# zhouxuguang/GNXRayTracer

Hardware: AMD Instinct MI355X
Metric: Mrays/sec + wall-clock to 1024spp, dragon Cornell 1920×1080 (higher is better)
Workload: dtype f32; 1 GPU; cfg3: Cornell + synthetic 100000-tri mesh (stand-in for absent dragon.3d), Glass+Metal, PathIntegrator maxDepth 8 rr 1 spatial, Halton(1024), 1920x1080; passes_in_flight=4, sub_passes=56, spp_rendered=1024, gather=n/a, world_size=1, backend=none, devices_visible=1

## Files before the change

### gnxraytracer_amd/csrc/api.hip

```cpp
#include <hip/hip_runtime.h>

#include <chrono>
#include <cstdio>
#include <cstdlib>
#include <memory>
#include <mutex>
#include <string>
#include <thread>
#include <vector>

#include "host_scene.h"
#include "kernels.hip.h"
#include "trace4_kernel.hip.h"
#include "hlbvh_build.hip.h"
#include "refit_kernel.hip.h"
#include "material_kernel.hip.h"
#include "rebuild_kernel.hip.h"
#include "li_kernel.hip.h"
#include "views_kernel.hip.h"
#include "shade_query_kernel.hip.h"
#include "aov_kernel.hip.h"
#include "kernel_instances.h"

using namespace gnxr;
// ... 25 lines not shown
int gnxr_init(int device_id) {
    int n = 0;
    hipError_t e = hipGetDeviceCount(&n);
    if (e != hipSuccess || n <= 0) { set_error("no HIP device available; libgnxr has no CPU fallback"); return GNXR_ERR_NO_DEVICE; }
    if (device_id < 0 || device_id >= n) { set_error("device %d out of range (%d visible)", device_id, n); return GNXR_ERR_INVALID; }
    HIP_TRY(hipSetDevice(device_id));
    g_device = -1;
    g_devices.assign(1, device_id);
    g_peer_ok.assign(1, 1);
    return ensure_device();
}
int gnxr_init_devices(int32_t n_devices, const int32_t *device_ids) {
    if (n_devices <= 0 || n_devices > 64 || !device_ids) { set_error("bad device list"); return GNXR_ERR_INVALID; }
    int n = 0;
    hipError_t e = hipGetDeviceCount(&n);
    if (e != hipSuccess || n <= 0) { set_error("no HIP device available; libgnxr has no CPU fallback"); return GNXR_ERR_NO_DEVICE; }
    for (int i = 0; i < n_devices; ++i)
        if (device_ids[i] < 0 || device_ids[i] >= n) { set_error("device %d out of range (%d visible)", device_ids[i], n); return GNXR_ERR_INVALID; }
    int rc = gnxr_init(device_ids[0]);
    if (rc) return rc;
    g_devices.assign(device_ids, device_ids + n_devices);
    g_peer_ok.assign(n_devices, 1);
    for (int i = 1; i < n_devices; ++i) {
        if (device_ids[i] == device_ids[0]) continue;
        int can01 = 0, can10 = 0;
        bool ok = hipDeviceCanAccessPeer(&can01, device_ids[0], device_ids[i]) == hipSuccess && can01 &&
                  hipDeviceCanAccessPeer(&can10, device_ids[i], device_ids[0]) == hipSuccess && can10;
        if (ok) {
            hipError_t e0 = hipSetDevice(device_ids[0]) == hipSuccess ? hipDeviceEnablePeerAccess(device_ids[i], 0) : hipErrorInvalidDevice;
            hipError_t e1 = hipSetDevice(device_ids[i]) == hipSuccess ? hipDeviceEnablePeerAccess(device_ids[0], 0) : hipErrorInvalidDevice;
            ok = (e0 == hipSuccess || e0 == hipErrorPeerAccessAlreadyEnabled) && (e1 == hipSuccess || e1 == hipErrorPeerAccessAlreadyEnabled);
        }
        g_peer_ok[i] = ok ? 1 : 0;
        if (getenv("GNXR_VERBOSE")) fprintf(stderr, "[gnxr] device %d <-> %d: %s\n", device_ids[0], device_ids[i], ok ? "peer access" : "no peer access: rows are staged through the host");
    }
    (void)hipGetLastError();
    if (getenv("GNXR_NO_PEER")) for (int i = 1; i < n_devices; ++i) g_peer_ok[i] = 0;
    HIP_TRY(hipSetDevice(device_ids[0]));
    return GNXR_OK;
}
void gnxr_shutdown(void) { g_device = -1; g_devices.clear(); g_peer_ok.clear(); }
int gnxr_set_profiling(int flags) { g_profiling = flags; return GNXR_OK; }
#ifdef GX_SHADE_STATS
int gnxr_debug_shade_stats(unsigned long long *out16, int reset) {
    if (hipMemcpyFromSymbol(out16, HIP_SYMBOL(g_shade_stats), 16 * sizeof(unsigned long long)) != hipSuccess) return GNXR_ERR_INVALID;
    if (reset) { unsigned long long z[16] = {0}; (void)hipMemcpyToSymbol(HIP_SYMBOL(g_shade_stats), z, sizeof(z)); }
    return GNXR_OK;
}
#endif
#ifdef GX_TRACE_STATS
int gnxr_debug_trace_stats(unsigned long long *out16, int reset) {
    if (hipMemcpyFromSymbol(out16, HIP_SYMBOL(g_trace_stats), 24 * sizeof(unsigned long long)) != hipSuccess) return GNXR_ERR_INVALID;
    if (reset) { unsigned long long z[24] = {0}; (void)hipMemcpyToSymbol(HIP_SYMBOL(g_trace_stats), z, sizeof(z)); }
    return GNXR_OK;
}
#endif

static int upload_scene(gnxr_scene *s, size_t) {
    const CompiledScene &cs = s->cs;
    int rc;
    if (cs.bvh_max_depth + 1 > 64) { set_error("BVH depth %d exceeds the 64-entry traversal stack (BVHAccel.cpp:661)", cs.bvh_max_depth); return GNXR_ERR_UNSUPPORTED; }
    s->set_traversal(std::any_of(cs.nodes.begin(), cs.nodes.end(), [](const DNode &n) { return (n.meta & 0xffffu) > 127; }));
#define UP(field) if ((rc = s->field.upload(cs.field)) != GNXR_OK) return rc;
    UP(nodes) UP(nodes4) UP(tris) UP(leaf_boxes) UP(tri_class) UP(lights) UP(perms) UP(primes) UP(prime_sums) UP(prime_magic)
    UP(dmedia) UP(grid_density) UP(tri_media) UP(spheres) UP(textures) UP(tex_texels) UP(ewa_lut) UP(tri_uv) UP(tri_n) UP(tri_s)
    UP(aov_albedo)
    UP(env_texels4) UP(env_cond_func) UP(env_cond_cdf) UP(env_cond_int) UP(env_marg_func) UP(env_marg_cdf) UP(env_marg_guide) UP(env_cond_guide)
#undef UP
    {
        const size_t worst = 2 * cs.desc_materials.size();
        if ((rc = s->material_authored.alloc(worst)) || (rc = s->materials.alloc(1 + worst)) || (rc = s->materials_single.alloc(1 + worst))) return rc;
        if ((rc = s->material_authored.upload(cs.material_authored)) != GNXR_OK) return rc;
        const DTexTables rec = s->tex_tables(s->tri_uv.p, s->tri_n.p, s->tri_s.p);
        for (int k = 0; k < 2; ++k) {
            const std::vector<DMaterial> &src = k == 0 ? cs.materials : cs.materials_single;
            std::vector<DMaterial> up(src.size() + 1);
            memset(&up[0], 0, sizeof(DMaterial));
            memcpy(&up[0], &rec, sizeof(rec));
            std::copy(src.begin(), src.end(), up.begin() + 1);
            if ((rc = (k == 0 ? s->materials : s->materials_single).upload(up)) != GNXR_OK) return rc;
        }
    }
    if ((rc = s->infinite.upload(cs.infinite_lights)) != GNXR_OK) return rc;
    if ((rc = s->counters.alloc(1)) != GNXR_OK) return rc;
    if (hipHostMalloc((void **)&s->h_counters, sizeof(Counters)) != hipSuccess) { set_error("hipHostMalloc failed"); return GNXR_ERR_OOM; }
    if (hipHostMalloc((void **)&s->h_ring, sizeof(Counters) * gnxr_scene::kRing) != hipSuccess) { set_error("hipHostMalloc failed"); return GNXR_ERR_OOM; }
    for (hipEvent_t &e : s->ring_ev) HIP_TRY(hipEventCreateWithFlags(&e, hipEventDisableTiming));
    for (hipStream_t &a : s->aux_stream) HIP_TRY(hipStreamCreateWithFlags(&a, hipStreamNonBlocking));
    HIP_TRY(hipEventCreateWithFlags(&s->ev_fork, hipEventDisableTiming));
    for (hipEvent_t &e : s->ev_join) HIP_TRY(hipEventCreateWithFlags(&e, hipEventDisableTiming));
    return GNXR_OK;
}

int gnxr_scene_create(const gnxr_scene_desc *desc, gnxr_scene **out) {
    if (!desc || !out) { set_error("null argument"); return GNXR_ERR_INVALID; }
    int rc = ensure_device();
    if (rc) return rc;
    gnxr_scene *s = new (std::nothrow) gnxr_scene(g_device);
    if (!s) return GNXR_ERR_OOM;
    if (!compile_scene(desc, &s->cs, device_hlbvh_build)) { delete s; return GNXR_ERR_INVALID; }
    for (size_t i = 1; i < g_devices.size(); ++i) s->replicas.push_back(std::make_unique<gnxr_scene>(g_devices[i], s->host));
    if ((rc = s->each_copy(upload_scene)) != GNXR_OK) { delete s; return rc; }
    const CompiledScene &cs = s->cs;
    if (getenv("GNXR_VERBOSE"))
        fprintf(stderr, "[gnxr] scene: %zu tris, %zu nodes (depth %d), %zu 4-wide nodes (stack %d), wide=%d, %zu device(s)\n", cs.tris.size(), cs.nodes.size(), cs.bvh_max_depth,
                cs.nodes4.size(), cs.stack4_need, (int)s->wide_ok, s->n_copies());
// ... 282 lines not shown
```

### gnxraytracer_amd/csrc/api_render.hip.h

```cpp
#pragma once

struct TraceLaunch {
    int entries;
    int lds_entries;
    bool spill_needed;
    size_t lds;
    int n_top;
    int blocks;
};
static TraceLaunch trace_launch(const gnxr_scene *s, bool wide, bool spheres, long long total) {
    TraceLaunch t;
    t.entries = wide ? s->cs.stack4_need + 1 : s->cs.bvh_max_depth + 2;
    const int per_cu = g_trace_blocks_per_cu;
    const size_t fixed_b = wide ? (size_t)(kRayRecDwords + (spheres ? 1 : 0)) * kRqStride * sizeof(int) + (size_t)kTopCache * 128 + 128 : 0;
    t.lds_entries = std::min(std::min(t.entries, Knobs::trace_lds_levels()), std::max(2, (int)(((160 * 1024) / per_cu - 1024 - fixed_b) / (kBlock * sizeof(int)))));
    t.spill_needed = t.entries > t.lds_entries;
    t.lds = (size_t)t.lds_entries * kBlock * sizeof(int) + fixed_b;
    t.n_top = (int)std::min<size_t>(kTopCache, s->cs.root4 >= 0 ? s->cs.nodes4.size() : 0);
    t.blocks = (int)std::min<long long>((long long)g_num_cus * per_cu, (total + kBlock - 1) / kBlock);
    return t;
}

static int count_local_rows(const gnxr_render_params *p) {
    int rows = 0;
// ... 220 lines not shown
VolPackSet RenderState::pack_set(bool alt) {
    VolPackSet ps;
    if (!alt) {
        float4 *a[kVolPackF4] = {L.p, reinterpret_cast<float4 *>(vol_vs.p), vol_n1.p, vol_f.p, vol_Li.p, vol_Tr.p, vol_Ld.p, mis_Y.p, vol_mres.p};
        for (int i = 0; i < kVolPackF4; ++i) ps.f4[i] = a[i];
        record_ptrs(rec, ps.rec);
        ps.state = vol_state.p; ps.orig = vol_orig.p;
    } else {
        for (int i = 0; i < kVolPackF4; ++i) ps.f4[i] = vol_alt[i].p;
        record_ptrs(vol_alt_rec, ps.rec);
        ps.state = vol_alt_state.p; ps.orig = vol_alt_orig.p;
    }
    return ps;
}

struct RenderRun {
    gnxr_scene *s;
    RenderState &st;
    hipStream_t stream;
    const RenderPlan &pl;
    const RaySource *src;
    const ViewSource *views;
    DScene sc;
    DRender r;
    PathArrays pa;
    VolArrays va;
    WhittedArrays wa;
    DMediaTables mt;
    Counters *dctr;
    KernelTimer timer;
    const bool timing = (g_profiling & 1) != 0, count_wide = (g_profiling & 4) != 0, counting = (g_profiling & 2) != 0 && !count_wide;
    bool spheres;
    bool list_media = false;
    int n_lights, n_scene_media;
    unsigned long long rays_closest = 0, rays_any = 0, rays_mis = 0, media_segments = 0;
    unsigned long long new_paths = 0;
    unsigned int launches = 0, passes = 0, loop_iterations = 0;

    RenderRun(gnxr_scene *scene, hipStream_t stream_, const RenderPlan &plan, const RaySource *src_, const ViewSource *views_, const DScene &sc_, const DRender &r_)
        : s(scene), st(scene->st), stream(stream_), pl(plan), src(src_), views(views_), sc(sc_), r(r_), pa(st.path_arrays()), va(st.vol_arrays()),
          wa(st.whitted_arrays(plan, (int)scene->cs.desc_lights.size())), mt(scene->media_tables()), dctr(scene->counters.p), spheres(scene->cs.n_spheres > 0),
          n_lights((int)scene->cs.desc_lights.size()), n_scene_media((int)scene->cs.media.size()) {}

    void launch_trace(TraceWork w, int n_sh, int n_mis, bool count_rays = true);
    void compact(int mode, const int *qin, int nin, const unsigned char *keys, int nout, int nscatter, unsigned int *totals, int *o0, int *o1, int *o2, int *o3 = nullptr, int split = 0,
                 const unsigned *n_dev = nullptr);
    int shade_stage(const int *q_in, int n, int *q_out, const unsigned *n_dev);
    void raygen(const PathArrays &at, long long u0, int kk, unsigned char *medium_keys);
    void resolve(const PathArrays &at, long long u0, int kk);
    void bind_set(const VolPackSet &ps);
};

void RenderRun::launch_trace(TraceWork w, int n_sh, int n_mis, bool count_rays) {
    long long total = (long long)w.n_closest + 2ll * w.n_nee;
    if (total <= 0) return;
    w.order = nullptr;
    (void)hipMemsetAsync(&dctr->cursor, 0, sizeof(unsigned int), stream);
    const bool wide = s->wide_ok && !counting;
    const TraceLaunch tl = trace_launch(s, wide, spheres, total);
    if (timing) timer.begin(0, stream);
    const int chunk = Knobs::trace_chunk();
#define GX_TRACE(C, W, S) hipLaunchKernelGGL((k_trace<C, W, S>), dim3(tl.blocks), dim3(kBlock), tl.lds, stream, sc, pa, w, &dctr->cursor, dctr, tl.lds_entries, st.trace_spill.p, chunk)
#define GX_TRACE4(C, S, P) hipLaunchKernelGGL((k_trace4<C, S, P>), dim3(tl.blocks), dim3(kBlock), tl.lds, stream, sc, pa, w, &dctr->cursor, dctr, tl.lds_entries, st.trace_spill.p, chunk, tl.n_top)
#define GX_TRACE4_CS(C, S) do { if (tl.spill_needed) GX_TRACE4(C, S, true); else GX_TRACE4(C, S, false); } while (0)
    if (wide) {
        if (spheres) { if (count_wide) GX_TRACE4_CS(true, true); else GX_TRACE4_CS(false, true); }
        else { if (count_wide) GX_TRACE4_CS(true, false); else GX_TRACE4_CS(false, false); }
    } else {
        const bool cnt = counting || count_wide;
        if (spheres) { if (cnt) GX_TRACE(true, false, true); else GX_TRACE(false, false, true); }
        else { if (cnt) GX_TRACE(true, false, false); else GX_TRACE(false, false, false); }
    }
#undef GX_TRACE4_CS
#undef GX_TRACE4
#undef GX_TRACE
    if (timing) timer.end(stream);
    if (count_rays) {
        rays_closest += (unsigned long long)w.n_closest + (unsigned long long)n_mis;
        rays_any += (unsigned long long)n_sh;
        rays_mis += (unsigned long long)n_mis;
    }
    ++launches;
}

void RenderRun::compact(int mode, const int *qin, int nin, const unsigned char *keys, int nout, int nscatter, unsigned int *totals, int *o0, int *o1, int *o2, int *o3, int split,
                        const unsigned *n_dev) {
    const int tiles = (nin + kCompactTile - 1) / kCompactTile;
    const int g = std::max(1, std::min(tiles, g_num_cus * kCompactBlocksPerCu));
    if (st.compact_seq >= (1u << 30) - 1u) {
        (void)hipMemsetAsync(st.tile_desc.p, 0, st.tile_desc.n * sizeof(unsigned long long), stream);
        st.compact_seq = 0;
    }
    const unsigned seq = ++st.compact_seq;
    const CompactScratch cs{st.tile_desc.p, tiles, st.compact_ticket.p + (seq & 1u), st.compact_ticket.p + ((seq + 1u) & 1u), seq};
    const bool hitclass = mode == COMPACT_HITCLASS;
    const int *hit = hitclass ? (const int *)st.hit.p : nullptr;
    const unsigned char *cls = hitclass ? (const unsigned char *)s->tri_class.p : nullptr;
#define GX_COMPACT(M, N, NS) hipLaunchKernelGGL((k_compact<M, N, NS>), dim3(g), dim3(kCompactBlock), 0, stream, qin, nin, keys, cs, totals, o0, o1, o2, o3, hit, cls, split, n_dev, dctr)
    if (mode == COMPACT_FLAGS) {
        if (nout == 5) { if (nscatter == 3) GX_COMPACT(COMPACT_FLAGS, 5, 3); else GX_COMPACT(COMPACT_FLAGS, 5, 2); }
        else { if (nscatter == 3) GX_COMPACT(COMPACT_FLAGS, 4, 3); else GX_COMPACT(COMPACT_FLAGS, 4, 2); }
    } else if (hitclass) { if (nout == 4) GX_COMPACT(COMPACT_HITCLASS, 4, 4); else GX_COMPACT(COMPACT_HITCLASS, 3, 3); }
    else if (nout == 4) GX_COMPACT(COMPACT_CLASS, 4, 4);
    else GX_COMPACT(COMPACT_CLASS, 3, 3);
#undef GX_COMPACT
    launches += 1;
}
// ... 557 lines not shown
```

### gnxraytracer_amd/csrc/trace4_kernel.hip.h

```cpp
#pragma once
#include "kernels.hip.h"
#include "query_kernel.hip.h"

namespace gnxr {

GX_DEV unsigned order_entry(unsigned code, unsigned hm) {
    const unsigned base0 = (code & 4u) ? 2u : 0u, sw0 = (code >> 1) & 1u, sw1 = code & 1u, base1 = 2u - base0;
    const unsigned ord[4] = {base0 + sw0, base0 + 1u - sw0, base1 + sw1, base1 + 1u - sw1};
    unsigned e = 0, n = 0;
    for (int i = 0; i < 4; ++i)
        if ((hm >> ord[i]) & 1u) { e |= ord[i] << (2u * n); ++n; }
    return e;
}
#ifndef GX_T4_CACHE
#define GX_T4_CACHE 64
#endif
constexpr int kTopCache = GX_T4_CACHE;
constexpr int kRayRecDwords = 11;
#ifndef GX_T4_RQ
#define GX_T4_RQ 64
#endif
constexpr int kRayQueue = GX_T4_RQ;
constexpr int kRqStride = (kBlock / 64) * kRayQueue;
GX_DEV int trace4_lds_dwords_per_thread(bool sph) { return kRayRecDwords + (sph ? 1 : 0); }

#ifndef GX_T4_WAVES
#define GX_T4_WAVES 5
#endif
#if GX_T4_WAVES > 0
#define GX_T4_BOUNDS __launch_bounds__(kBlock, GX_T4_WAVES)
#else
#define GX_T4_BOUNDS __launch_bounds__(kBlock)
#endif
template <bool COUNT, bool SPH, bool SPILL, int Q = kT4Render>
__global__ void GX_T4_BOUNDS k_trace4(DScene sc, typename Trace4Src<Q>::type pa, TraceWork w, unsigned int *cursor, Counters *ctr, int lds_entries, int *spill, int chunk, int n_top) {
    extern __shared__ int smem[];
    typedef __attribute__((address_space(3))) float lds_float;
    lds_int *const stk = (lds_int *)&smem[threadIdx.x];
    global_int *const spl = (global_int *)(spill + (size_t)blockIdx.x * kBlock + threadIdx.x);
    const int spillStride = (int)gridDim.x * kBlock;
    const int lane = __lane_id();
    lds_int *const rq = (lds_int *)&smem[lds_entries * kBlock + (threadIdx.x >> 6) * kRayQueue];
    trace_work_counts(w);
    const unsigned total = (unsigned)w.n_closest + 2u * (unsigned)w.n_nee;
    chunk = trace_chunk(total, chunk);
    const ChunkPlan plan = chunk_plan(total, (unsigned)chunk);
    const unsigned nWaves = gridDim.x * (kBlock / 64u), waveId = blockIdx.x * (kBlock / 64u) + (threadIdx.x >> 6);
    bool firstFetch = true;
    const DTri *__restrict__ tris = sc.tris;
    const char *__restrict__ nb = reinterpret_cast<const char *>(sc.nodes4);
    typedef float f4v __attribute__((ext_vector_type(4)));
    typedef __attribute__((address_space(3))) f4v lds_f4;
    typedef __attribute__((address_space(3))) unsigned char lds_u8;
    lds_f4 *const topN = (lds_f4 *)&smem[lds_entries * kBlock + (kRayRecDwords + (SPH ? 1 : 0)) * kRqStride];
    lds_u8 *const lut = (lds_u8 *)(topN + 8 * kTopCache);
    {
        const f4v *gn = reinterpret_cast<const f4v *>(sc.nodes4);
        for (int i = threadIdx.x; i < n_top * 8; i += kBlock) topN[(i & 7) * kTopCache + (i >> 3)] = gn[i];
        if (threadIdx.x < 128) lut[threadIdx.x] = (unsigned char)order_entry(threadIdx.x >> 4, threadIdx.x & 15u);
        __syncthreads();
    }

    auto push = [&](int &n, int v) {
        if (!SPILL || n < lds_entries) stk[n * kBlock] = v;
        else spl[(n - lds_entries) * spillStride] = v;
        ++n;
    };
    auto pop = [&](int &n) -> int {
        --n;
        return (!SPILL || n < lds_entries) ? stk[n * kBlock] : spl[(n - lds_entries) * spillStride];
    };

#ifndef GX_T4_REFILL_IN_A
#define GX_T4_REFILL_IN_A 0
#endif
    unsigned poolBase = 0, poolCount = 0;
    bool exhausted = false;
    unsigned rqHead = 0, rqCount = 0;

    bool live = false;
    int pk = 0, path = -1;
    V3 ro, inv;
    float Sx = 0, Sy = 0, tMax = 0;
    unsigned oNX = 0, oNY = 16, oNZ = 32;
    unsigned ordShift = 0;
    int cur = -1, toVisit = 0, leafOff = 0, leafN = 0, hitLeaf = -1;
    uint32_t cntNodes = 0, cntTris = 0, cntRetests = 0, cntNodesGlobal = 0;
#ifdef GX_TRACE_STATS
    unsigned long long st_[24] = {0};
#endif

    auto take_ray = [&](unsigned slot) {
        const lds_float *q = (const lds_float *)(rq + slot);
        ro = V3(q[0 * kRqStride], q[1 * kRqStride], q[2 * kRqStride]); tMax = q[3 * kRqStride];
        inv = V3(q[4 * kRqStride], q[5 * kRqStride], q[6 * kRqStride]); Sx = q[7 * kRqStride];
        Sy = q[8 * kRqStride];
        pk = __float_as_int(q[9 * kRqStride]);
        path = __float_as_int(q[10 * kRqStride]);
        hitLeaf = SPH ? rq[slot + 11 * kRqStride] : -1;
        const int neg0 = inv.x < 0, neg1 = inv.y < 0, neg2 = inv.z < 0;
        oNX = neg0 ? 48u : 0u; oNY = neg1 ? 64u : 16u; oNZ = neg2 ? 80u : 32u;
        ordShift = 8u * (unsigned)(neg0 | (neg1 << 1) | (neg2 << 2));
        cur = ((pk >> 4) & 1) ? -1 : sc.root4; toVisit = 0; leafN = 0;
        live = true;
    };
    auto retire_ray = [&]() {
        const int kind = pk & 3;
        if constexpr (Q == kT4QueryClosest) pa.hits[path].prim = hitLeaf;
        else if constexpr (Q == kT4QueryAny) pa.occluded[path] = hitLeaf != -1 ? 1 : 0;
        else if (kind == 0) {
            pa.hit[path] = hitLeaf;
            if (hitLeaf < 0) {
                int cls = sc.escape_class;
                if (SPH && hitLeaf != -1) { const int mat = sc.spheres[-2 - hitLeaf].material; if (mat >= 0) cls = sc.materials[mat].shade_class; }
                else if (sc.lt.n_infinite == 0) {
                    cls = 4;
                    pa.pflags[path] = 0;
                }
                pa.pclass[path] = (unsigned char)cls;
            }
        }
        else if (kind == 1) {
            if (w.vis) w.vis[4 * (size_t)path] = hitLeaf == -1 ? 1 : 0;
            else reinterpret_cast<float *>(&pa.sh_o[(size_t)path * kRS])[3] = hitLeaf == -1 ? 1.f : 0.f;
        } else {
            const int expect = __float_as_int(pa.mis_o[(size_t)path * kRS].w);
            bool ok = (expect >= 0) ? (hitLeaf == expect) : (hitLeaf == -1);
            if (w.vis) w.vis[4 * (size_t)path + 1] = ok ? 1 : 0;
            else reinterpret_cast<float *>(&pa.mis_o[(size_t)path * kRS])[3] = ok ? 1.f : 0.f;
        }
        live = false;
    };
#ifdef GX_TRACE_STATS
#define GX_TICK(i) do { const unsigned long long t_ = __builtin_amdgcn_s_memtime(); GX_STAT(i, t_ - tick_); tick_ = t_; } while (0)
    unsigned long long tick_ = __builtin_amdgcn_s_memtime();
#else
#define GX_TICK(i) do {} while (0)
#endif
    while (true) {
        GX_STAT(0, 1);
        GX_TICK(15);
        const bool need = !live;
        const unsigned long long needMask = __ballot(need);
        if (needMask) {
            if (rqCount == 0) {
                if (poolCount == 0 && !exhausted) {
                    unsigned v = waveId;
                    if (!firstFetch) {
                        if (lane == 0) v = nWaves + atomicAdd(cursor, 1u);
                        v = __shfl(v, 0);
                    }
                    firstFetch = false;
                    if (!chunk_range(plan, v, total, &poolBase, &poolCount)) { exhausted = true; poolCount = 0; }
                }
                if (poolCount > 0) {
                    const unsigned take = min(poolCount, (unsigned)kRayQueue);
                    bool valid = false;
                    float4 r0 = make_float4(0, 0, 0, 0), r1 = r0, r2 = r0;
                    int sphHit = -1;
                    if ((unsigned)lane < take) {
                        unsigned i = poolBase + (unsigned)lane;
                        if (w.order) i = w.order[i];
                        float4 o4, d4;
                        int kind_ = 0, path_, any_ = 0;
                        float tMax_;
                        valid = true;
                        if constexpr (Q != kT4Render) {
                            path_ = (int)i;
                            o4 = pa.rays[2 * (size_t)i]; d4 = pa.rays[2 * (size_t)i + 1];
                            tMax_ = o4.w;
                            kind_ = Q == kT4QueryAny ? 1 : 0; any_ = kind_;
                        } else if (i < (unsigned)w.n_closest) {
                            path_ = w.q_closest ? w.q_closest[i] : (int)i;
                            o4 = pa.ray_o[(size_t)path_ * kRS]; d4 = pa.ray_d[(size_t)path_ * kRS];
                            tMax_ = o4.w;
                        } else {
                            const unsigned e = i - (unsigned)w.n_closest;
                            const bool isShadow = e < (unsigned)w.n_nee;
                            path_ = w.q_nee[isShadow ? e : e - (unsigned)w.n_nee];
                            const bool together = w.vis != nullptr;
                            if (isShadow) {
                                kind_ = 1; any_ = 1;
                                o4 = pa.sh_o[(size_t)path_ * kRS]; d4 = pa.sh_d[(size_t)path_ * kRS]; tMax_ = o4.w;
                                valid = (__float_as_int(d4.w) & 1) != 0;
                            } else {
                                kind_ = 2;
                                const int nflags = __float_as_int(pa.sh_d[(size_t)path_ * kRS].w);
                                valid = (nflags & 2) != 0;
                                if (together || valid) { o4 = pa.mis_o[(size_t)path_ * kRS]; d4 = pa.mis_d[(size_t)path_ * kRS]; }
                                else { o4 = make_float4(0, 0, 0, 0); d4 = o4; }
                                tMax_ = GX_INF;
                                any_ = __float_as_int(o4.w) < 0 ? 1 : 0;
                            }
                        }
                        if (valid) {
                            const V3 o(o4.x, o4.y, o4.z), d(d4.x, d4.y, d4.z);
                            const V3 iv(1.f / d.x, 1.f / d.y, 1.f / d.z);
                            const RayShear sh = ray_shear(d);
                            int done = 0;
                            for (int si = 0; SPH && si < sc.n_spheres; ++si) {
                                float tH;
                                if (sphere_test(sc.spheres[si], o, d, tMax_, &tH)) {
                                    sphHit = -2 - si;
                                    if (any_) { done = 1; break; }
                                    tMax_ = tH;
                                }
                            }
                            const int ex = (__builtin_isinf(iv.x) || __builtin_isinf(iv.y) || __builtin_isinf(iv.z)) ? 1 : 0;
                            r0 = make_float4(o.x, o.y, o.z, tMax_);
                            r1 = make_float4(iv.x, iv.y, iv.z, sh.Sx);
                            r2 = make_float4(sh.Sy, __int_as_float(kind_ | (sh.kz << 2) | (done << 4) | (ex << 5) | (any_ << 6)), __int_as_float(path_), 0.f);
                        }
                    }
                    const unsigned long long vm = __ballot(valid);
                    if (valid) {
                        const int slot = __popcll(vm & ((1ull << lane) - 1ull));
                        lds_float *q = (lds_float *)(rq + slot);
                        q[0 * kRqStride] = r0.x; q[1 * kRqStride] = r0.y; q[2 * kRqStride] = r0.z; q[3 * kRqStride] = r0.w;
                        q[4 * kRqStride] = r1.x; q[5 * kRqStride] = r1.y; q[6 * kRqStride] = r1.z; q[7 * kRqStride] = r1.w;
                        q[8 * kRqStride] = r2.x; q[9 * kRqStride] = r2.y; q[10 * kRqStride] = r2.z;
                        if (SPH) rq[slot + 11 * kRqStride] = sphHit;
                    }
                    __builtin_amdgcn_fence(__ATOMIC_SEQ_CST, "wavefront");
                    rqCount = (unsigned)__popcll(vm); rqHead = 0;
                    poolBase += take; poolCount -= take;
                    GX_STAT(7, 1);
                    GX_STAT(8, take);
                }
            }
            if (rqCount > 0) {
                const unsigned rank = (unsigned)__popcll(needMask & ((1ull << lane) - 1ull));
                if (need && rank < rqCount) take_ray(rqHead + rank);
                const unsigned t = min(rqCount, (unsigned)__popcll(needMask));
                rqHead += t; rqCount -= t;
                __builtin_amdgcn_fence(__ATOMIC_SEQ_CST, "wavefront");
            }
        }
        GX_TICK(11);
        const unsigned long long liveMask = __ballot(live);
        if (liveMask == 0) {
            if (exhausted && rqCount == 0 && poolCount == 0) break;
            continue;
        }

        int nLive = __popcll(liveMask);
        GX_STAT(9, nLive);
        while (true) {
#if GX_T4_REFILL_IN_A
            {
                const bool fin = live && cur == -1 && leafN == 0;
                const unsigned long long finMask = __ballot(fin);
                if (finMask != 0 && rqCount > 0) {
                    if (fin) retire_ray();
                    const unsigned rank = (unsigned)__popcll(finMask & ((1ull << lane) - 1ull));
                    if (fin && rank < rqCount) take_ray(rqHead + rank);
                    const unsigned t = min(rqCount, (unsigned)__popcll(finMask));
                    rqHead += t; rqCount -= t;
                    __builtin_amdgcn_fence(__ATOMIC_SEQ_CST, "wavefront");
                    nLive = __popcll(__ballot(live));
                }
            }
#endif
            if (live && leafN == 0 && cur < -1) {
                const int lr = ~cur;
                leafOff = lr & 0xffffff; leafN = (lr >> 24) & 0x7f;
                cur = (toVisit == 0) ? -1 : pop(toVisit);
            }
            const bool searching = live && cur >= 0 && (kSpeculate || leafN == 0);
            const bool hungry = searching && leafN == 0;
            const int nSearching = __popcll(__ballot(hungry));
            if (nSearching * kTraceLeaveDiv <= nLive * kTraceLeaveMul && (nSearching == 0 || nSearching < nLive)) break;
#ifdef GX_TRACE_STATS
            { const int ns = __popcll(__ballot(searching)); GX_STAT(1, 1); GX_STAT(2, ns); const int nh_ = __popcll(__ballot(live && leafN > 0 && !searching)), nf_ = __popcll(__ballot(live && cur == -1 && leafN == 0)), nsp_ = __popcll(__ballot(searching && leafN > 0));
              GX_STAT(20, nLive); GX_STAT(21, nh_); GX_STAT(22, nf_); GX_STAT(23, nsp_);
              const int n16 = __popcll(__ballot(searching && cur < 16)), n64 = __popcll(__ballot(searching && cur < 64)), n256 = __popcll(__ballot(searching && cur < 256)), n1k = __popcll(__ballot(searching && cur < 1024));
              GX_STAT(16, n16); GX_STAT(17, n64); GX_STAT(18, n256); GX_STAT(19, n1k); }
#endif
            if (searching) {
                if (COUNT) cntNodes++;
                f4v nX, fX, nY, fY, nZ, fZ, cf;
// ... 75 lines not shown
                GX_STAT(3, 1); GX_STAT(4, __popcll(lm)); GX_STAT(5, mx); GX_STAT(6, sm); GX_STAT(10, nre);
            }
        }
#endif
        if (live && leafN > 0) {
            bool visit = true;
            const bool first = (pk & 128) == 0;
            const bool retest = first && (SPH ? hitLeaf != -1 : hitLeaf >= 0);
            const bool fromVerts = retest && leafN == 1 && sc.leaf1_from_verts;
            int neg[3] = {inv.x < 0, inv.y < 0, inv.z < 0};
            if (retest && !fromVerts) {
                const float4 b0 = sc.leaf_box[2 * (size_t)leafOff], b1 = sc.leaf_box[2 * (size_t)leafOff + 1];
                if (COUNT) cntRetests++;
                visit = slab_test(b0, b1, ro, inv, neg, tMax);
            }
            bool more = false;
            if (visit) {
                RayShear shear;
                const int kz = (pk >> 2) & 3;
                shear.kz = kz; shear.kx = kz == 2 ? 0 : kz + 1; shear.ky = shear.kx == 2 ? 0 : shear.kx + 1;
                shear.Sx = Sx; shear.Sy = Sy; shear.Sz = kz == 0 ? inv.x : (kz == 1 ? inv.y : inv.z);
                V3 p0, p1, p2;
                load_tri(tris, leafOff, &p0, &p1, &p2);
                if (COUNT) cntTris++;
                bool inBox = true;
                if (fromVerts) {
                    const float4 b0 = make_float4(fminf(fminf(p0.x, p1.x), p2.x), fminf(fminf(p0.y, p1.y), p2.y), fminf(fminf(p0.z, p1.z), p2.z), fmaxf(fmaxf(p0.x, p1.x), p2.x));
                    const float4 b1 = make_float4(fmaxf(fmaxf(p0.y, p1.y), p2.y), fmaxf(fmaxf(p0.z, p1.z), p2.z), 0.f, 0.f);
                    inBox = slab_test(b0, b1, ro, inv, neg, tMax);
                }
                more = leafN > 1;
                TriHit h;
                if (inBox && tri_test_sheared(p0, p1, p2, ro, shear, tMax, &h)) {
                    hitLeaf = leafOff;
                    if (pk & 64) { cur = -1; more = false; }
                    else tMax = h.t;
                }
            }
            if (more) { leafOff += 1; leafN -= 1; pk |= 128; }
            else { leafN = 0; pk &= ~128; }
        }
        GX_TICK(13);
        if (live && cur == -1 && leafN == 0) retire_ray();
    }
#ifdef GX_TRACE_STATS
    if (lane == 0) for (int i = 0; i < 24; ++i) if (st_[i]) atomicAdd(&g_trace_stats[i], st_[i]);
#endif
    if (COUNT) {
        atomicAdd(&ctr->nodes, (unsigned long long)cntNodes);
        atomicAdd(&ctr->tris, (unsigned long long)cntTris);
        atomicAdd(&ctr->retests, (unsigned long long)cntRetests);
        atomicAdd(&ctr->nodes_global, (unsigned long long)cntNodesGlobal);
    }
}

}
```

### gnxraytracer_amd/csrc/trace_kernel.hip.h

```cpp
#pragma once
#include "device_geom.h"

namespace gnxr {

struct TraceWork {
    const int *q_closest; int n_closest;
    const int *q_nee; int n_nee;
    const unsigned *order;
    unsigned char *vis;
    const unsigned *n_closest_dev, *n_nee_dev;
};
GX_DEV void trace_work_counts(TraceWork &w) {
    if (w.n_closest_dev) { w.n_closest = (int)*w.n_closest_dev; w.n_nee = w.n_nee_dev ? (int)*w.n_nee_dev : 0; }
}
GX_DEV int trace_chunk(unsigned total, int chunk_max) {
    const unsigned waves = gridDim.x * (blockDim.x / 64u);
    const unsigned per = ((total + waves - 1u) / waves + 63u) / 64u * 64u;
    return (int)min((unsigned)chunk_max, max(64u, per));
}

struct ChunkPlan { unsigned c, big, k1, mid_end, k2; };
GX_DEV ChunkPlan chunk_plan(unsigned total, unsigned c) {
    const unsigned waves = gridDim.x * (blockDim.x / 64u);
    ChunkPlan p;
    p.c = c;
    const unsigned tail = waves * 384u;
    p.big = (c > 128u && total > tail) ? (total - tail) / c * c : 0u;
    p.k1 = p.big / c;
    const unsigned mid = min(total - p.big, waves * 256u) / 128u * 128u;
    p.mid_end = p.big + mid;
    p.k2 = mid / 128u;
    return p;
}
GX_DEV bool chunk_range(const ChunkPlan &p, unsigned v, unsigned total, unsigned *base, unsigned *count) {
    unsigned b, n;
    if (v < p.k1) { b = v * p.c; n = p.c; }
    else if (v < p.k1 + p.k2) { b = p.big + (v - p.k1) * 128u; n = 128u; }
    else {
        const unsigned long long bb = (unsigned long long)p.mid_end + (unsigned long long)(v - p.k1 - p.k2) * 64ull;
        if (bb >= total) return false;
        b = (unsigned)bb; n = 64u;
    }
    if (b >= total) return false;
    *base = b; *count = min(n, total - b);
    return true;
}

constexpr int kTraceChunk = 512;
#ifndef GX_TRACE_LEAVE_MUL
#define GX_TRACE_LEAVE_MUL 1
#endif
#ifndef GX_TRACE_LEAVE_DIV
#define GX_TRACE_LEAVE_DIV 2
#endif
#ifndef GX_REFILL_MIN
#define GX_REFILL_MIN 1
#endif
#ifndef GX_SPECULATE
#define GX_SPECULATE 1
#endif
constexpr bool kSpeculate = GX_SPECULATE != 0;
#ifndef GX_NEE_INTERLEAVED
#define GX_NEE_INTERLEAVED 0
#endif
constexpr int kRefillMin = GX_REFILL_MIN;
constexpr int kTraceLeaveMul = GX_TRACE_LEAVE_MUL, kTraceLeaveDiv = GX_TRACE_LEAVE_DIV;

typedef __attribute__((address_space(3))) int lds_int;
typedef __attribute__((address_space(1))) int global_int;
struct LaneStack {
    lds_int *lds;
    global_int *spill;
    int K;
    int stride;
    GX_DEV void push(int &n, int v) const {
        if (n < K) lds[n * kBlock] = v;
        else spill[(n - K) * stride] = v;
        ++n;
    }
    GX_DEV int pop(int &n) const {
        --n;
        return n < K ? lds[n * kBlock] : spill[(n - K) * stride];
    }
};

struct RayOctant {
    int nx, fx, ny, fy, nz, fz;
    int shift;
};
GX_DEV RayOctant ray_octant(int neg0, int neg1, int neg2) {
    RayOctant r;
    r.nx = neg0 ? 3 : 0; r.fx = 3 - r.nx;
    r.ny = neg1 ? 4 : 1; r.fy = 5 - r.ny;
    r.nz = neg2 ? 5 : 2; r.fz = 7 - r.nz;
    r.shift = 8 * (neg0 | (neg1 << 1) | (neg2 << 2));
    return r;
}

GX_DEV int bvh4_step(const float4 *__restrict__ n4, int node, V3 ro, V3 invDir, const RayOctant &oc, float tMaxRay, const LaneStack &stack, int &toVisit) {
    const float4 *q = n4 + 8 * (size_t)node;
    const float4 nX = q[oc.nx], fX = q[oc.fx], nY = q[oc.ny], fY = q[oc.fy], nZ = q[oc.nz], fZ = q[oc.fz];
    const float4 cf = q[6], mf = q[7];
    const float k = 1 + 2 * GX_GAMMA(3);
    unsigned hitMask = 0;
#define GX_SLAB(C, BIT)                                                                   \
    {                                                                                     \
        float tMin = (nX.C - ro.x) * invDir.x, tMax = (fX.C - ro.x) * invDir.x;           \
        float tyMin = (nY.C - ro.y) * invDir.y, tyMax = (fY.C - ro.y) * invDir.y;         \
        tMax *= k; tyMax *= k;                                                            \
        bool ok = !(tMin > tyMax || tyMin > tMax);                                        \
        if (tyMin > tMin) tMin = tyMin;                                                   \
        if (tyMax < tMax) tMax = tyMax;                                                   \
        float tzMin = (nZ.C - ro.z) * invDir.z, tzMax = (fZ.C - ro.z) * invDir.z;         \
        tzMax *= k;                                                                       \
        ok = ok && !(tMin > tzMax || tzMin > tMax);                                       \
        if (tzMin > tMin) tMin = tzMin;                                                   \
        if (tzMax < tMax) tMax = tzMax;                                                   \
        ok = ok && (tMin < tMaxRay) && (tMax > 0);                                        \
        hitMask |= ok ? (BIT) : 0u;                                                       \
    }
    GX_SLAB(x, 1u) GX_SLAB(y, 2u) GX_SLAB(z, 4u) GX_SLAB(w, 8u)
#undef GX_SLAB
    if (hitMask == 0) return (toVisit == 0) ? kRefDone : stack.pop(toVisit);
    const unsigned long long table = ((unsigned long long)__float_as_uint(mf.y) << 32) | __float_as_uint(mf.x);
    const unsigned ord = (unsigned)(table >> oc.shift);
    const int c0 = __float_as_int(cf.x), c1 = __float_as_int(cf.y), c2 = __float_as_int(cf.z), c3 = __float_as_int(cf.w);
    int next = kRefDone;
    bool have = false;
#pragma unroll
    for (int kk = 3; kk >= 0; --kk) {
        const unsigned slot = (ord >> (2 * kk)) & 3u;
        if ((hitMask >> slot) & 1u) {
            if (have) stack.push(toVisit, next);
            next = slot == 0 ? c0 : (slot == 1 ? c1 : (slot == 2 ? c2 : c3));
            have = true;
        }
    }
    return next;
}

#ifdef GX_TRACE_STATS
static __device__ unsigned long long g_trace_stats[24];
#define GX_STAT(i, v) do { if (lane == 0) st_[i] += (unsigned long long)(v); } while (0)
#else
#define GX_STAT(i, v) do {} while (0)
#endif

template <bool COUNT, bool WIDE, bool SPH>
__global__ void __launch_bounds__(kBlock) k_trace(DScene sc, PathArrays pa, TraceWork w, unsigned int *cursor, Counters *ctr, int lds_entries, int *spill, int chunk) {
    extern __shared__ int stack_mem[];
    LaneStack stack;
    stack.lds = (lds_int *)&stack_mem[threadIdx.x];
    stack.K = lds_entries;
    stack.stride = (int)gridDim.x * kBlock;
    stack.spill = (global_int *)(spill + (size_t)blockIdx.x * kBlock + threadIdx.x);
    const int lane = __lane_id();
    trace_work_counts(w);
    const unsigned total = (unsigned)w.n_closest + 2u * (unsigned)w.n_nee;
    chunk = trace_chunk(total, chunk);
    const float4 *__restrict__ nodes = sc.nodes;
    const DTri *__restrict__ tris = sc.tris;

    unsigned poolBase = 0, poolCount = 0;
    bool exhausted = false;

    int item = -1, kind = 0, path = -1;
    V3 ro, rd, invDir;
    RayShear shear;
    RayOctant oct = ray_octant(0, 0, 0);
    float tMax = 0;
    int neg0 = 0, neg1 = 0, neg2 = 0;
    int cur = -1, toVisit = 0, leafOff = 0, leafN = 0, hitLeaf = -1, expect = -1;
    uint32_t cntNodes = 0, cntTris = 0, cntRetests = 0;
#ifdef GX_TRACE_STATS
    unsigned long long st_[24] = {0};
#endif

    while (true) {
        GX_STAT(0, 1);
        bool need = item < 0;
        unsigned long long needMask = __ballot(need);
        if (kRefillMin > 1 && __popcll(needMask) < kRefillMin && needMask != ~0ull) needMask = 0;
        if (needMask) {
            GX_STAT(7, 1);
            GX_STAT(8, __popcll(needMask));
            if (poolCount == 0 && !exhausted) {
                unsigned base = 0;
                if (lane == 0) base = atomicAdd(cursor, (unsigned)chunk);
                base = __shfl(base, 0);
                if (base >= total) exhausted = true;
                else { poolBase = base; poolCount = min((unsigned)chunk, total - base); }
            }
            if (poolCount > 0) {
                unsigned rank = (unsigned)__popcll(needMask & ((1ull << lane) - 1ull));
                unsigned take = min(poolCount, (unsigned)__popcll(needMask));
                if (need && rank < take) {
                    unsigned i = poolBase + rank;
                    if (w.order) i = w.order[i];
                    item = (int)i;
                    float4 o4, d4;
                    if (i < (unsigned)w.n_closest) {
                        kind = 0;
                        path = w.q_closest ? w.q_closest[i] : (int)i;
                        o4 = pa.ray_o[(size_t)path * kRS]; d4 = pa.ray_d[(size_t)path * kRS];
                        tMax = o4.w;
                    } else {
                        unsigned e = i - (unsigned)w.n_closest;
                        const bool isShadow = GX_NEE_INTERLEAVED ? (e & 1u) == 0 : e < (unsigned)w.n_nee;
                        path = w.q_nee[GX_NEE_INTERLEAVED ? (e >> 1) : (isShadow ? e : e - (unsigned)w.n_nee)];
                        int nflags = __float_as_int(pa.sh_d[(size_t)path * kRS].w);
                        if (isShadow) {
                            kind = 1;
                            if (nflags & 1) { o4 = pa.sh_o[(size_t)path * kRS]; d4 = pa.sh_d[(size_t)path * kRS]; tMax = o4.w; }
                            else item = -1;
                        } else {
                            kind = 2;
                            if (nflags & 2) { o4 = pa.mis_o[(size_t)path * kRS]; d4 = pa.mis_d[(size_t)path * kRS]; expect = __float_as_int(o4.w); tMax = GX_INF; }
                            else item = -1;
                        }
                    }
                    if (item >= 0) {
                        ro = V3(o4.x, o4.y, o4.z); rd = V3(d4.x, d4.y, d4.z);
                        invDir = V3(1.f / rd.x, 1.f / rd.y, 1.f / rd.z);
                        shear = ray_shear(rd);
                        neg0 = invDir.x < 0; neg1 = invDir.y < 0; neg2 = invDir.z < 0;
                        if (WIDE) oct = ray_octant(neg0, neg1, neg2);
                        cur = WIDE ? sc.root4 : 0; toVisit = 0; leafN = 0; hitLeaf = -1;
                        for (int si = 0; SPH && si < sc.n_spheres; ++si) {
                            float tH;
                            if (sphere_test(sc.spheres[si], ro, rd, tMax, &tH)) {
                                hitLeaf = -2 - si;
                                if (kind == 1) { cur = -1; break; }
                                tMax = tH;
                            }
                        }
                    }
                }
                poolBase += take; poolCount -= take;
            }
        }
        if (__ballot(item >= 0) == 0) {
            if (exhausted) break;
            continue;
        }

        const int nLive = __popcll(__ballot(item >= 0));
        GX_STAT(9, nLive);
        while (true) {
            if (WIDE && item >= 0 && leafN == 0 && cur < -1) {
                int lr = ~cur;
                leafOff = lr & 0xffffff; leafN = (lr >> 24) & 0x7f;
                cur = (toVisit == 0) ? -1 : stack.pop(toVisit);
            }
            bool searching = item >= 0 && cur >= 0 && (kSpeculate && WIDE ? true : leafN == 0);
            bool hungry = searching && leafN == 0;
            int nSearching = __popcll(__ballot(hungry));
            if (nSearching * kTraceLeaveDiv <= nLive * kTraceLeaveMul && (nSearching == 0 || nSearching < nLive)) break;
            GX_STAT(1, 1);
            GX_STAT(2, __popcll(__ballot(searching)));
            if (searching) {
                if (COUNT) cntNodes++;
                if (WIDE) {
                    int next = bvh4_step(sc.nodes4, cur, ro, invDir, oct, tMax, stack, toVisit);
                    cur = (next == kRefDone) ? -1 : next;
                } else {
                    float4 n0 = nodes[2 * cur], n1 = nodes[2 * cur + 1];
                    int neg[3] = {neg0, neg1, neg2};
                    bool hitBox = slab_test(n0, n1, ro, invDir, neg, tMax);
                    int offset = __float_as_int(n1.z);
                    uint32_t meta = __float_as_uint(n1.w);
                    int nPrims = (int)(meta & 0xffffu);
                    int next;
// ... 108 lines not shown
```

Before: 4968 Mrays/s.

## Fetch shadow and MIS rays per NEE work item instead of separate items

The trace work-item space changes from n_closest + 2*n_nee to n_closest + n_nee. Each NEE item now loads its flags once, traces the shadow ray and, if a MIS ray is needed, traces it from the same lane as a second pass. In the wide kernel a wave holds the pool and runs an extra MIS pass before advancing. This removes the redundant flag loads and the empty lanes for paths lacking a shadow or MIS ray, but it adds per-lane serialization and divergence when only some lanes owe a MIS ray. Optional tail-timing instrumentation and chunk-size macros are also added.

```diff
diff --git a/gnxraytracer_amd/csrc/api.hip b/gnxraytracer_amd/csrc/api.hip
--- a/gnxraytracer_amd/csrc/api.hip
+++ b/gnxraytracer_amd/csrc/api.hip
@@ -101,6 +101,13 @@
 int gnxr_debug_trace_stats(unsigned long long *out16, int reset) {
     if (hipMemcpyFromSymbol(out16, HIP_SYMBOL(g_trace_stats), 24 * sizeof(unsigned long long)) != hipSuccess) return GNXR_ERR_INVALID;
     if (reset) { unsigned long long z[24] = {0}; (void)hipMemcpyToSymbol(HIP_SYMBOL(g_trace_stats), z, sizeof(z)); }
+    return GNXR_OK;
+}
+#endif
+#ifdef GX_TAIL_STAMP
+int gnxr_debug_tail_stamp(unsigned long long *out12, int reset) {
+    if (hipMemcpyFromSymbol(out12, HIP_SYMBOL(g_tail), 12 * sizeof(unsigned long long)) != hipSuccess) return GNXR_ERR_INVALID;
+    if (reset) { unsigned long long z[12] = {~0ull, 0ull, ~0ull, 0ull}; (void)hipMemcpyToSymbol(HIP_SYMBOL(g_tail), z, sizeof(z)); }
     return GNXR_OK;
 }
 #endif
diff --git a/gnxraytracer_amd/csrc/api_render.hip.h b/gnxraytracer_amd/csrc/api_render.hip.h
--- a/gnxraytracer_amd/csrc/api_render.hip.h
+++ b/gnxraytracer_amd/csrc/api_render.hip.h
@@ -296,7 +296,7 @@
 };
 
 void RenderRun::launch_trace(TraceWork w, int n_sh, int n_mis, bool count_rays) {
-    long long total = (long long)w.n_closest + 2ll * w.n_nee;
+    long long total = (long long)w.n_closest + w.n_nee;
     if (total <= 0) return;
     w.order = nullptr;
     (void)hipMemsetAsync(&dctr->cursor, 0, sizeof(unsigned int), stream);
diff --git a/gnxraytracer_amd/csrc/trace4_kernel.hip.h b/gnxraytracer_amd/csrc/trace4_kernel.hip.h
--- a/gnxraytracer_amd/csrc/trace4_kernel.hip.h
+++ b/gnxraytracer_amd/csrc/trace4_kernel.hip.h
@@ -42,11 +42,16 @@
     const int lane = __lane_id();
     lds_int *const rq = (lds_int *)&smem[lds_entries * kBlock + (threadIdx.x >> 6) * kRayQueue];
     trace_work_counts(w);
-    const unsigned total = (unsigned)w.n_closest + 2u * (unsigned)w.n_nee;
+    const unsigned total = (unsigned)w.n_closest + (unsigned)w.n_nee;
     chunk = trace_chunk(total, chunk);
     const ChunkPlan plan = chunk_plan(total, (unsigned)chunk);
     const unsigned nWaves = gridDim.x * (kBlock / 64u), waveId = blockIdx.x * (kBlock / 64u) + (threadIdx.x >> 6);
     bool firstFetch = true;
+#ifdef GX_TAIL_STAMP
+    const unsigned tailFrom = total;
+    bool tailSeen = false;
+    if (Q == kT4Render && waveId == 0 && lane == 0) atomicMin(&g_tail[2], (unsigned long long)wall_clock64());
+#endif
     const DTri *__restrict__ tris = sc.tris;
     const char *__restrict__ nb = reinterpret_cast<const char *>(sc.nodes4);
     typedef float f4v __attribute__((ext_vector_type(4)));
@@ -80,6 +85,7 @@
 
     bool live = false;
     int pk = 0, path = -1;
+    constexpr int kMisOwed = 256;
     V3 ro, inv;
     float Sx = 0, Sy = 0, tMax = 0;
     unsigned oNX = 0, oNY = 16, oNZ = 32;
@@ -95,7 +101,7 @@
         ro = V3(q[0 * kRqStride], q[1 * kRqStride], q[2 * kRqStride]); tMax = q[3 * kRqStride];
         inv = V3(q[4 * kRqStride], q[5 * kRqStride], q[6 * kRqStride]); Sx = q[7 * kRqStride];
         Sy = q[8 * kRqStride];
-        pk = __float_as_int(q[9 * kRqStride]);
+        pk = (pk & kMisOwed) | __float_as_int(q[9 * kRqStride]);
         path = __float_as_int(q[10 * kRqStride]);
         hitLeaf = SPH ? rq[slot + 11 * kRqStride] : -1;
         const int neg0 = inv.x < 0, neg1 = inv.y < 0, neg2 = inv.z < 0;
@@ -144,7 +150,8 @@
         const unsigned long long needMask = __ballot(need);
         if (needMask) {
             if (rqCount == 0) {
-                if (poolCount == 0 && !exhausted) {
+                const bool misPass = Q == kT4Render && __ballot((pk & kMisOwed) != 0) != 0;
+                if (!misPass && poolCount == 0 && !exhausted) {
                     unsigned v = waveId;
                     if (!firstFetch) {
                         if (lane == 0) v = nWaves + atomicAdd(cursor, 1u);
@@ -152,13 +159,19 @@
                     }
                     firstFetch = false;
                     if (!chunk_range(plan, v, total, &poolBase, &poolCount)) { exhausted = true; poolCount = 0; }
-                }
-                if (poolCount > 0) {
+#ifdef GX_TAIL_STAMP
+                    if (Q == kT4Render && !tailSeen && (exhausted || poolBase + poolCount >= tailFrom)) {
+                        tailSeen = true;
+                        if (lane == 0) atomicMin(&g_tail[0], (unsigned long long)wall_clock64());
+                    }
+#endif
+                }
+                if (misPass || poolCount > 0) {
                     const unsigned take = min(poolCount, (unsigned)kRayQueue);
-                    bool valid = false;
+                    bool valid = false, wantMis = false;
                     float4 r0 = make_float4(0, 0, 0, 0), r1 = r0, r2 = r0;
                     int sphHit = -1;
-                    if ((unsigned)lane < take) {
+                    if (misPass ? (pk & kMisOwed) != 0 : (unsigned)lane < take) {
                         unsigned i = poolBase + (unsigned)lane;
                         if (w.order) i = w.order[i];
                         float4 o4, d4;
@@ -175,20 +188,16 @@
                             o4 = pa.ray_o[(size_t)path_ * kRS]; d4 = pa.ray_d[(size_t)path_ * kRS];
                             tMax_ = o4.w;
                         } else {
-                            const unsigned e = i - (unsigned)w.n_closest;
-                            const bool isShadow = e < (unsigned)w.n_nee;
-                            path_ = w.q_nee[isShadow ? e : e - (unsigned)w.n_nee];
-                            const bool together = w.vis != nullptr;
-                            if (isShadow) {
+                            path_ = w.q_nee[i - (unsigned)w.n_closest];
+                            if (!misPass) {
                                 kind_ = 1; any_ = 1;
                                 o4 = pa.sh_o[(size_t)path_ * kRS]; d4 = pa.sh_d[(size_t)path_ * kRS]; tMax_ = o4.w;
-                                valid = (__float_as_int(d4.w) & 1) != 0;
+                                const int nflags = __float_as_int(d4.w);
+                                valid = (nflags & 1) != 0;
+                                wantMis = (nflags & 2) != 0;
                             } else {
                                 kind_ = 2;
-                                const int nflags = __float_as_int(pa.sh_d[(size_t)path_ * kRS].w);
-                                valid = (nflags & 2) != 0;
-                                if (together || valid) { o4 = pa.mis_o[(size_t)path_ * kRS]; d4 = pa.mis_d[(size_t)path_ * kRS]; }
-                                else { o4 = make_float4(0, 0, 0, 0); d4 = o4; }
+                                o4 = pa.mis_o[(size_t)path_ * kRS]; d4 = pa.mis_d[(size_t)path_ * kRS];
                                 tMax_ = GX_INF;
                                 any_ = __float_as_int(o4.w) < 0 ? 1 : 0;
                             }
@@ -223,9 +232,15 @@
                     }
                     __builtin_amdgcn_fence(__ATOMIC_SEQ_CST, "wavefront");
                     rqCount = (unsigned)__popcll(vm); rqHead = 0;
-                    poolBase += take; poolCount -= take;
+                    bool advance = true;
+                    if (Q == kT4Render) {
+                        if (misPass) pk &= ~kMisOwed;
+                        else if (wantMis) pk |= kMisOwed;
+                        advance = misPass || __ballot(wantMis) == 0;
+                    }
+                    if (advance) { poolBase += take; poolCount -= take; }
                     GX_STAT(7, 1);
-                    GX_STAT(8, take);
+                    GX_STAT(8, misPass ? rqCount : take);
                 }
             }
             if (rqCount > 0) {
@@ -407,6 +422,21 @@
         atomicAdd(&ctr->retests, (unsigned long long)cntRetests);
         atomicAdd(&ctr->nodes_global, (unsigned long long)cntNodesGlobal);
     }
+#ifdef GX_TAIL_STAMP
+    if (Q == kT4Render && lane == 0) {
+        atomicMax(&g_tail[1], (unsigned long long)wall_clock64());
+        __threadfence();
+        if (atomicAdd(&g_tail[3], 1ull) == (unsigned long long)nWaves - 1ull) {
+            __threadfence();
+            const unsigned long long tEnd = atomicExch(&g_tail[1], 0ull), tCross = atomicExch(&g_tail[0], ~0ull), tStart = atomicExch(&g_tail[2], ~0ull);
+            atomicExch(&g_tail[3], 0ull);
+            const unsigned long long behind = tEnd > tCross ? tEnd - tCross : 0ull, all = tEnd > tStart ? tEnd - tStart : 0ull;
+            const int o = total >= (1u << 24) ? 8 : 4;
+            g_tail[o] += behind; g_tail[o + 1] += all; g_tail[o + 2] += 1ull; g_tail[o + 3] += total;
+            if (o == 8) { g_tail[4] += behind; g_tail[5] += all; g_tail[6] += 1ull; g_tail[7] += total; }
+        }
+    }
+#endif
 }
 
 }
diff --git a/gnxraytracer_amd/csrc/trace_kernel.hip.h b/gnxraytracer_amd/csrc/trace_kernel.hip.h
--- a/gnxraytracer_amd/csrc/trace_kernel.hip.h
+++ b/gnxraytracer_amd/csrc/trace_kernel.hip.h
@@ -19,15 +19,21 @@
     return (int)min((unsigned)chunk_max, max(64u, per));
 }
 
+#ifndef GX_CHUNK_TAIL
+#define GX_CHUNK_TAIL 384
+#endif
+#ifndef GX_CHUNK_MID
+#define GX_CHUNK_MID 256
+#endif
 struct ChunkPlan { unsigned c, big, k1, mid_end, k2; };
 GX_DEV ChunkPlan chunk_plan(unsigned total, unsigned c) {
     const unsigned waves = gridDim.x * (blockDim.x / 64u);
     ChunkPlan p;
     p.c = c;
-    const unsigned tail = waves * 384u;
+    const unsigned tail = waves * (unsigned)GX_CHUNK_TAIL;
     p.big = (c > 128u && total > tail) ? (total - tail) / c * c : 0u;
     p.k1 = p.big / c;
-    const unsigned mid = min(total - p.big, waves * 256u) / 128u * 128u;
+    const unsigned mid = min(total - p.big, waves * (unsigned)GX_CHUNK_MID) / 128u * 128u;
     p.mid_end = p.big + mid;
     p.k2 = mid / 128u;
     return p;
@@ -60,9 +66,6 @@
 #define GX_SPECULATE 1
 #endif
 constexpr bool kSpeculate = GX_SPECULATE != 0;
-#ifndef GX_NEE_INTERLEAVED
-#define GX_NEE_INTERLEAVED 0
-#endif
 constexpr int kRefillMin = GX_REFILL_MIN;
 constexpr int kTraceLeaveMul = GX_TRACE_LEAVE_MUL, kTraceLeaveDiv = GX_TRACE_LEAVE_DIV;
 
@@ -146,6 +149,10 @@
 #define GX_STAT(i, v) do {} while (0)
 #endif
 
+#ifdef GX_TAIL_STAMP
+static __device__ unsigned long long g_tail[12] = {~0ull, 0ull, ~0ull, 0ull, 0ull, 0ull, 0ull, 0ull, 0ull, 0ull, 0ull, 0ull};
+#endif
+
 template <bool COUNT, bool WIDE, bool SPH>
 __global__ void __launch_bounds__(kBlock) k_trace(DScene sc, PathArrays pa, TraceWork w, unsigned int *cursor, Counters *ctr, int lds_entries, int *spill, int chunk) {
     extern __shared__ int stack_mem[];
@@ -156,7 +163,7 @@
     stack.spill = (global_int *)(spill + (size_t)blockIdx.x * kBlock + threadIdx.x);
     const int lane = __lane_id();
     trace_work_counts(w);
-    const unsigned total = (unsigned)w.n_closest + 2u * (unsigned)w.n_nee;
+    const unsigned total = (unsigned)w.n_closest + (unsigned)w.n_nee;
     chunk = trace_chunk(total, chunk);
     const float4 *__restrict__ nodes = sc.nodes;
     const DTri *__restrict__ tris = sc.tris;
@@ -165,6 +172,7 @@
     bool exhausted = false;
 
     int item = -1, kind = 0, path = -1;
+    int misPath = -1;
     V3 ro, rd, invDir;
     RayShear shear;
     RayOctant oct = ray_octant(0, 0, 0);
@@ -179,45 +187,51 @@
     while (true) {
         GX_STAT(0, 1);
         bool need = item < 0;
-        unsigned long long needMask = __ballot(need);
-        if (kRefillMin > 1 && __popcll(needMask) < kRefillMin && needMask != ~0ull) needMask = 0;
-        if (needMask) {
+        const bool second = need && misPath >= 0;
+        const unsigned long long secondMask = __ballot(second);
+        unsigned long long needMask = __ballot(need && !second);
+        if (kRefillMin > 1 && __popcll(needMask) < kRefillMin && (needMask | secondMask) != ~0ull) needMask = 0;
+        if (needMask | secondMask) {
             GX_STAT(7, 1);
-            GX_STAT(8, __popcll(needMask));
-            if (poolCount == 0 && !exhausted) {
+            GX_STAT(8, __popcll(needMask | secondMask));
+            if (needMask && poolCount == 0 && !exhausted) {
                 unsigned base = 0;
                 if (lane == 0) base = atomicAdd(cursor, (unsigned)chunk);
                 base = __shfl(base, 0);
                 if (base >= total) exhausted = true;
                 else { poolBase = base; poolCount = min((unsigned)chunk, total - base); }
             }
-            if (poolCount > 0) {
+            {
                 unsigned rank = (unsigned)__popcll(needMask & ((1ull << lane) - 1ull));
                 unsigned take = min(poolCount, (unsigned)__popcll(needMask));
-                if (need && rank < take) {
-                    unsigned i = poolBase + rank;
-                    if (w.order) i = w.order[i];
-                    item = (int)i;
+                if (second || (need && rank < take)) {
                     float4 o4, d4;
-                    if (i < (unsigned)w.n_closest) {
-                        kind = 0;
-                        path = w.q_closest ? w.q_closest[i] : (int)i;
-                        o4 = pa.ray_o[(size_t)path * kRS]; d4 = pa.ray_d[(size_t)path * kRS];
-                        tMax = o4.w;
-                    } else {
-                        unsigned e = i - (unsigned)w.n_closest;
-                        const bool isShadow = GX_NEE_INTERLEAVED ? (e & 1u) == 0 : e < (unsigned)w.n_nee;
-                        path = w.q_nee[GX_NEE_INTERLEAVED ? (e >> 1) : (isShadow ? e : e - (unsigned)w.n_nee)];
-                        int nflags = __float_as_int(pa.sh_d[(size_t)path * kRS].w);
-                        if (isShadow) {
-                            kind = 1;
-                            if (nflags & 1) { o4 = pa.sh_o[(size_t)path * kRS]; d4 = pa.sh_d[(size_t)path * kRS]; tMax = o4.w; }
-                            else item = -1;
+                    bool mis = second;
+                    if (second) { path = misPath; item = 0; }
+                    else {
+                        unsigned i = poolBase + rank;
+                        if (w.order) i = w.order[i];
+                        item = (int)i;
+                        if (i < (unsigned)w.n_closest) {
+                            kind = 0;
+                            path = w.q_closest ? w.q_closest[i] : (int)i;
+                            o4 = pa.ray_o[(size_t)path * kRS]; d4 = pa.ray_d[(size_t)path * kRS];
+                            tMax = o4.w;
                         } else {
-                            kind = 2;
-                            if (nflags & 2) { o4 = pa.mis_o[(size_t)path * kRS]; d4 = pa.mis_d[(size_t)path * kRS]; expect = __float_as_int(o4.w); tMax = GX_INF; }
+                            path = w.q_nee[i - (unsigned)w.n_closest];
+                            const int nflags = __float_as_int(pa.sh_d[(size_t)path * kRS].w);
+                            if (nflags & 1) {
+                                kind = 1;
+                                o4 = pa.sh_o[(size_t)path * kRS]; d4 = pa.sh_d[(size_t)path * kRS]; tMax = o4.w;
+                                if (nflags & 2) misPath = path;
+                            }
+                            else if (nflags & 2) mis = true;
                             else item = -1;
                         }
+                    }
+                    if (mis) {
+                        kind = 2; misPath = -1;
+                        o4 = pa.mis_o[(size_t)path * kRS]; d4 = pa.mis_d[(size_t)path * kRS]; expect = __float_as_int(o4.w); tMax = GX_INF;
                     }
                     if (item >= 0) {
                         ro = V3(o4.x, o4.y, o4.z); rd = V3(d4.x, d4.y, d4.z);
```

New measurement: 5092 Mrays/s (median of 6 runs). 2.5% higher.
